# elun15/Graph-Convolutional-Network-for-Multi-Camera-Vehicle-Tracking

Measured on NVIDIA B200. Metric: mpn_inference_directed_edges_per_sec, higher is better.
Workload: dtype f32

## Files before the change

graph-convolutional-network-for-multi-camera-vehicle-tracking_b200/csrc/mpn_forward.cu:

```cuda
#include <mutex>
#include <new>
#include <stdlib.h>
#include <string.h>

#include "common.cuh"
#include "kernels.h"
#include "tcgen05.cuh"

namespace mpn {

enum {
  FC_ENC1_W = 0,
  FC_ENC1_C = 8,
  FC_ENC2_W = 12,
  FC_ENC2_C = 28,
  FC_EDGE_WE = 32,
  FC_BN3_S = 48,
  FC_BN3_T = 52,
  FC_NODE_WE = 64,
  FC_BN4_S = 192,
  FC_BN4_T = 224,
  FC_CLS_W = 256,
  FC_CLS_B = 264,
  FC_EDGE_WE0 = 272,
  FC_TOTAL = 288
};

constexpr int SUMS = MPN_SUMS_DOUBLES;
constexpr int SWEEP_THREADS = 256;
constexpr int SWEEP_BLOCKS_PER_SM = 4;
constexpr int SWEEP_GRID = kNumSMs * SWEEP_BLOCKS_PER_SM;
constexpr int SWEEP_RESIDENT_BLOCKS = 3;
constexpr int SWEEP_RESIDENT_GRID = kNumSMs * SWEEP_RESIDENT_BLOCKS;
constexpr float BN_EPS = 1e-5f;

struct EdgeConsts {
  float v[FC_TOTAL];
};

__device__ __forceinline__ void load_consts(EdgeConsts& sc, const float* __restrict__ consts) {
  for (int i = threadIdx.x; i < FC_TOTAL; i += blockDim.x) sc.v[i] = consts[i];
  __syncthreads();
}

constexpr int TASK_PART = 16;
__device__ __forceinline__ void warp_load_consts(EdgeConsts& sc, const float* __restrict__ consts_g, int lane) {
  __syncwarp();
  for (int i = lane; i < FC_TOTAL; i += 32) sc.v[i] = consts_g[i];
  __syncwarp();
}

__device__ __forceinline__ void enc_layer1(const EdgeConsts& sc, float2 ea, float (&a1)[4]) {
#pragma unroll
  for (int j = 0; j < 4; ++j)
    a1[j] = fmaxf(fmaf(sc.v[FC_ENC1_W + 2 * j], ea.x, fmaf(sc.v[FC_ENC1_W + 2 * j + 1], ea.y, sc.v[FC_ENC1_C + j])), 0.f);
}
__device__ __forceinline__ void enc_layer2_pre(const float* __restrict__ w2 , const float* __restrict__ c2,
                                               const float (&a1)[4], float (&u)[4]) {
#pragma unroll
  for (int j = 0; j < 4; ++j) {
// ... 494 lines not shown
    const float a_row = BATCHED ? 0.f : A[(size_t)tr.row * MPN_DH + lane];
    const float4 ps = (YSRC == 0) ? Ps[tr.row] : make_float4(0.f, 0.f, 0.f, 0.f);
    float s1[4] = {0.f, 0.f, 0.f, 0.f};
    float q[10] = {0.f, 0.f, 0.f, 0.f, 0.f, 0.f, 0.f, 0.f, 0.f, 0.f};
    for (int base = tr.beg; base < tr.end; base += 32 * U) {
      EdgeLoad<U> L;
      load_edges<U, YSRC == 0, YSRC == 0, YSRC == 1>(L, g, base, tr.end, lane, edge_attr, Pd, ybuf);
#pragma unroll
      for (int j = 0; j < U; ++j) {
        float ep[4];
        eprime_of<YSRC>(sc, ps, L.ea[j], L.pd[j], L.y[j], ep);
        if (!L.ok[j]) { ep[0] = ep[1] = ep[2] = ep[3] = 0.f; }
        int idx = 0;
#pragma unroll
        for (int a = 0; a < 4; ++a) {
          s1[a] += ep[a];
#pragma unroll
          for (int b = a; b < 4; ++b) { q[idx] = fmaf(ep[a], ep[b], q[idx]); ++idx; }
        }
      }
    }
#pragma unroll
    for (int a = 0; a < 4; ++a) s1[a] = warp_sum(s1[a]);
    if (lane == 0) s1_task[t] = make_float4(s1[0], s1[1], s1[2], s1[3]);
    if (!BATCHED) {
      const float nt = (float)(tr.end - tr.beg);
      const float4 wn = *reinterpret_cast<const float4*>(small + MPN_W_NODE_W + lane * 36 + 32);
      const float qd = fmaf(wn.x, s1[0], fmaf(wn.y, s1[1], fmaf(wn.z, s1[2], wn.w * s1[3])));
      m1 += (double)fmaf(nt, a_row, qd);
      m2 += (double)(a_row * fmaf(nt, a_row, 2.0f * qd));
    }
#pragma unroll
    for (int i = 0; i < 10; ++i) {
      const double v = warp_sum((double)q[i]);
      if (BATCHED) { if (lane == 0) partials[(size_t)t * TASK_PART + i] = v; }
      else if (lane == i) t2 += v;
    }
    tp.rotate(row_nn);
  }
  if (!BATCHED) {
    const int warp = threadIdx.x >> 5;
    red_m[warp][lane] = m1;
    red_m[warp][32 + lane] = m2;
    block_sum_lane_columns<10, SWEEP_THREADS>(t2, red, partials + (size_t)blockIdx.x * SUMS + 64);
    if (threadIdx.x < 64) {
      double sm = 0.0;
      for (int wv = 0; wv < SWEEP_THREADS / 32; ++wv) sm += red_m[wv][threadIdx.x];
      partials[(size_t)blockIdx.x * SUMS + threadIdx.x] = sm;
    }
    finalize_in_last_block(fin);
  }
}

template <bool MAXOP = false>
__device__ __forceinline__ float transpose_reduce32(float (&acc)[32], int lane) {
#pragma unroll
  for (int o = 16, n = 16; o > 0; o >>= 1, n >>= 1) {
    const bool upper = (lane & o) != 0;
#pragma unroll
    for (int i = 0; i < 16; ++i) {
      if (i < n) {
        const float send = upper ? acc[i] : acc[i + n];
        const float keep = upper ? acc[i + n] : acc[i];
        const float other = __shfl_xor_sync(0xffffffffu, send, o);
        acc[i] = MAXOP ? fmaxf(keep, other) : keep + other;
      }
    }
  }
  return acc[0];
}

typedef unsigned long long f32x2;
__device__ __forceinline__ f32x2 pack2(float lo, float hi) {
  f32x2 r;
  asm("mov.b64 %0, {%1, %2};" : "=l"(r) : "f"(lo), "f"(hi));
  return r;
}
__device__ __forceinline__ void unpack2(f32x2 v, float& lo, float& hi) { asm("mov.b64 {%0, %1}, %2;" : "=f"(lo), "=f"(hi) : "l"(v)); }
__device__ __forceinline__ f32x2 fma2(f32x2 a, f32x2 b, f32x2 c) {
  f32x2 d;
  asm("fma.rn.f32x2 %0, %1, %2, %3;" : "=l"(d) : "l"(a), "l"(b), "l"(c));
  return d;
}
__device__ __forceinline__ f32x2 add2(f32x2 a, f32x2 b) {
  f32x2 d;
  asm("add.rn.f32x2 %0, %1, %2;" : "=l"(d) : "l"(a), "l"(b));
  return d;
}
__device__ __forceinline__ f32x2 relu2(f32x2 v) {
  float lo, hi;
  unpack2(v, lo, hi);
  return pack2(fmaxf(lo, 0.f), fmaxf(hi, 0.f));
}

__global__ void __launch_bounds__(SWEEP_THREADS, 2) enc_moments1_packed_kernel(const float4* __restrict__ edge_attr2, long long n_pairs,
                                                                             const float2* __restrict__ edge_attr, long long E,
                                                                             const float* __restrict__ consts, const float* __restrict__ small,
                                                                             double* __restrict__ partials, const FinArgs fin) {
  pdl_wait();
  __shared__ EdgeConsts sc;
  __shared__ double red[(SWEEP_THREADS / 32) * 8];
  load_consts(sc, consts);
  f32x2 w1x[4], w1y[4], c1[4], w2[16], c2[4];
#pragma unroll
  for (int j = 0; j < 4; ++j) {
    w1x[j] = pack2(sc.v[FC_ENC1_W + 2 * j], sc.v[FC_ENC1_W + 2 * j]);
    w1y[j] = pack2(sc.v[FC_ENC1_W + 2 * j + 1], sc.v[FC_ENC1_W + 2 * j + 1]);
    c1[j] = pack2(sc.v[FC_ENC1_C + j], sc.v[FC_ENC1_C + j]);
    const float b = small[MPN_W_ENC2_B + j];
    c2[j] = pack2(b, b);
#pragma unroll
    for (int k = 0; k < 4; ++k) { const float w = small[MPN_W_ENC2_W + 4 * j + k]; w2[4 * j + k] = pack2(w, w); }
  }
// ... 126 lines not shown
      acc[p] = 0ull;
    }
    EdgeLoad<U> cur, nxt;
    load_edges<U, YSRC == 0, YSRC == 0, YSRC == 1>(cur, g, tr.beg, tr.end, lane, edge_attr, Pd, ybuf);
    for (int base = tr.beg; base < tr.end; base += 32 * U) {
      const int nbase = base + 32 * U;
      if (nbase < tr.end) load_edges<U, YSRC == 0, YSRC == 0, YSRC == 1>(nxt, g, nbase, tr.end, lane, edge_attr, Pd, ybuf);
      float ep[U][4];
      f32x2 ed[U][4];
#pragma unroll
      for (int j = 0; j < U; ++j) {
        eprime_of<YSRC>(sc, ps, cur.ea[j], cur.pd[j], cur.y[j], ep[j]);
#pragma unroll
        for (int k = 0; k < 4; ++k) ed[j][k] = pack2(ep[j][k], ep[j][k]);
      }
#pragma unroll
      for (int p = 0; p < 16; ++p) {
        ulonglong2 wa, wb;
        asm volatile("ld.shared.v2.b64 {%0, %1}, [%2];" : "=l"(wa.x), "=l"(wa.y) : "r"(w2_addr + p * 32));
        asm volatile("ld.shared.v2.b64 {%0, %1}, [%2];" : "=l"(wb.x), "=l"(wb.y) : "r"(w2_addr + p * 32 + 16));
#pragma unroll
        for (int j = 0; j < U; ++j) {
          f32x2 z = fma2(wa.x, ed[j][0], ap[p]);
          z = fma2(wa.y, ed[j][1], z);
          z = fma2(wb.x, ed[j][2], z);
          z = fma2(wb.y, ed[j][3], z);
          z = relu2(z);
          if (cur.ok[j]) {
            if (AGGMAX) {
              float zl, zh, al, ah;
              unpack2(z, zl, zh);
              unpack2(acc[p], al, ah);
              acc[p] = pack2(fmaxf(al, zl), fmaxf(ah, zh));
            } else {
              acc[p] = add2(acc[p], z);
            }
          }
        }
      }
#pragma unroll
      for (int j = 0; j < U; ++j)
        if (cur.ok[j]) classify_store<CLASSIFY>(sc, ep[j], cur.e[j], logits, pred, prob1);
#pragma unroll
      for (int j = 0; j < U; ++j) {
        cur.e[j] = nxt.e[j];
        cur.ok[j] = nxt.ok[j];
        if (YSRC == 0) { cur.ea[j] = nxt.ea[j]; cur.pd[j] = nxt.pd[j]; }
        else cur.y[j] = nxt.y[j];
      }
    }
    float accf[32];
#pragma unroll
    for (int p = 0; p < 16; ++p) unpack2(acc[p], accf[2 * p], accf[2 * p + 1]);
    const float total = transpose_reduce32<AGGMAX>(accf, lane);
    msg_task[(size_t)t * MPN_DH + lane] = total;
  }
}

constexpr int ATC_THREADS = 128;
constexpr int ATC_CTAS_PER_SM = 5;
constexpr int ATC_SEG = 128;
constexpr int ATC_BATCHES = 512;
constexpr int ATC_NB = 2;
constexpr int ATC_D = 4;
constexpr int ATC_RL = ATC_D + 1;
constexpr int ATC_SLOT_BYTES = 128 * 16;
__device__ __forceinline__ int tile_off(int row, int kcore) { return (row >> 3) * 64 + kcore * 32 + (row & 7) * 4; }
constexpr int ATC_GROUP_BYTES = 3 * 128;
constexpr int ATC_TILE_BYTES = 16 * ATC_GROUP_BYTES;
__device__ __forceinline__ void split_tf32(float v, float& hi, float& lo) {
  hi = __uint_as_float((__float_as_uint(v) + 0x1000u) & 0xffffe000u);
  lo = v - hi;
}
template <int BYTES>
__device__ __forceinline__ void cp_async(void* smem_dst, const void* gsrc) {
  asm volatile("cp.async.ca.shared.global [%0], [%1], %2;" ::"r"(smem_u32(smem_dst)), "l"(gsrc), "n"(BYTES) : "memory");
}
__device__ __forceinline__ void cp_async_commit() { asm volatile("cp.async.commit_group;" ::: "memory"); }
template <int N>
__device__ __forceinline__ void cp_async_wait() { asm volatile("cp.async.wait_group %0;" ::"n"(N) : "memory"); }
__device__ __forceinline__ uint32_t opaque_u32(uint32_t v) {
  asm volatile("" : "+r"(v));
  return v;
}
__device__ __forceinline__ void sts128(uint32_t addr, float a, float b, float c, float d) {
  asm volatile("st.shared.v4.f32 [%0], {%1, %2, %3, %4};" ::"r"(addr), "f"(a), "f"(b), "f"(c), "f"(d) : "memory");
}
__device__ __forceinline__ float4 lds128(uint32_t addr) {
  float4 v;
  asm volatile("ld.shared.v4.f32 {%0, %1, %2, %3}, [%4];" : "=f"(v.x), "=f"(v.y), "=f"(v.z), "=f"(v.w) : "r"(addr) : "memory");
  return v;
}

template <bool CLASSIFY, bool DECIDE, bool AGGMAX, int CTAS>
__global__ void __launch_bounds__(ATC_THREADS, CTAS) apply_tc_kernel(
    const mpn_graph g, const float4* __restrict__ ybuf, const float* __restrict__ A, const float* __restrict__ consts,
    float* __restrict__ msg_task, float2* __restrict__ logits, uint8_t* __restrict__ pred, float* __restrict__ prob1) {
  pdl_wait();
  __shared__ EdgeConsts sc;
  __shared__ __align__(128) float et[2 * ATC_NB][ATC_TILE_BYTES / 4];
  __shared__ __align__(128) float w1[32 * 8];
  __shared__ __align__(128) float w2[32 * 8];
  __shared__ __align__(16) float4 ring[ATC_RL][ATC_THREADS];
  __shared__ int s_row[ATC_SEG], s_beg[ATC_SEG], s_end[ATC_SEG];
  __shared__ int s_bstart[ATC_BATCHES], s_nbatch;
  __shared__ float red[2][ATC_THREADS / 32][32];
  __shared__ __align__(8) uint64_t bar;
  __shared__ uint32_t tmem_slot;
  load_consts(sc, consts);
  const int tid = threadIdx.x, lane = tid & 31, warp = tid >> 5;
  if (warp == 0) tmem_alloc(&tmem_slot, 32 * ATC_NB);
  if (tid == 0) {
    mbar_init(&bar, 1);
    asm volatile("fence.mbarrier_init.release.cluster;" ::: "memory");
  }
  if (tid < 32) {
    float wh[4], wl[4];
#pragma unroll
    for (int k = 0; k < 4; ++k) {
      split_tf32(sc.v[FC_NODE_WE + 4 * tid + k], wh[k], wl[k]);
      uint32_t lb;
      asm("cvt.rna.tf32.f32 %0, %1;" : "=r"(lb) : "f"(wl[k]));
      wl[k] = __uint_as_float(lb);
    }
    *reinterpret_cast<float4*>(&w1[tile_off(tid, 0)]) = make_float4(wh[0], wh[1], wh[2], wh[3]);
    *reinterpret_cast<float4*>(&w1[tile_off(tid, 1)]) = make_float4(wh[0], wh[1], wh[2], wh[3]);
    *reinterpret_cast<float4*>(&w2[tile_off(tid, 0)]) = make_float4(wl[0], wl[1], wl[2], wl[3]);
    *reinterpret_cast<float4*>(&w2[tile_off(tid, 1)]) = make_float4(0.f, 0.f, 0.f, 0.f);
  }
  tc_fence_before();
  __syncthreads();
  tc_fence_after();
  const uint32_t tmem = tmem_slot;
  constexpr uint32_t IDESC = make_idesc_tf32(128, 32);
  const uint64_t d_w1 = make_smem_desc_noswizzle(smem_u32(w1), 128, 256), d_w2 = make_smem_desc_noswizzle(smem_u32(w2), 128, 256);
  const uint64_t d_e1 = make_smem_desc_noswizzle(smem_u32(et[0]), 128, ATC_GROUP_BYTES);
  const uint64_t d_e2 = make_smem_desc_noswizzle(smem_u32(et[0]) + 128, 128, ATC_GROUP_BYTES);
  constexpr uint64_t BUF_STEP = ATC_TILE_BYTES >> 4;
  const uint32_t my_tmem = opaque_u32(tmem + ((uint32_t)(warp * 32) << 16));
  const uint32_t et_addr = opaque_u32(smem_u32(et[0]) + (uint32_t)((tid >> 3) * ATC_GROUP_BYTES + (tid & 7) * 16));
  const uint32_t ring_addr = opaque_u32(smem_u32(&ring[0][tid]));
  constexpr uint32_t TILE_BYTES = ATC_TILE_BYTES;
#pragma unroll
  for (int i = 0; i < 2 * ATC_NB; ++i)
    sts128(et_addr + (uint32_t)i * TILE_BYTES + 256, 1.f, 1.f, 0.f, 0.f);
  uint32_t phase = 0;
  const int n_tasks = *g.n_tasks;
  const int per = (n_tasks + (int)gridDim.x - 1) / (int)gridDim.x;
  const int t_first = blockIdx.x * per, t_last = min(n_tasks, t_first + per);
  const float bn_s = sc.v[FC_BN4_S + lane], bn_t = sc.v[FC_BN4_T + lane];
  const float s3[4] = {sc.v[FC_BN3_S], sc.v[FC_BN3_S + 1], sc.v[FC_BN3_S + 2], sc.v[FC_BN3_S + 3]};
  const float t3[4] = {sc.v[FC_BN3_T], sc.v[FC_BN3_T + 1], sc.v[FC_BN3_T + 2], sc.v[FC_BN3_T + 3]};
  int flushes = 0;

  const int seg_tasks = min(ATC_SEG, ATC_BATCHES / max(1, g.chunk / ATC_THREADS));
  for (int s0 = t_first; s0 < t_last; s0 += seg_tasks) {
    const int ns = min(seg_tasks, t_last - s0);
    __syncthreads();
    for (int i = tid; i < ns; i += ATC_THREADS) {
      const TaskRange tr = task_range(g, s0 + i);
      s_row[i] = tr.row; s_beg[i] = tr.beg; s_end[i] = tr.end;
    }
    __syncthreads();
    for (int i = tid; i < ns; i += ATC_THREADS) {
      int first = 0;
      for (int k = 0; k < i; ++k) first += (s_end[k] - s_beg[k] + ATC_THREADS - 1) / ATC_THREADS;
      const int nb_i = (s_end[i] - s_beg[i] + ATC_THREADS - 1) / ATC_THREADS;
      for (int k = 0; k < nb_i; ++k) s_bstart[first + k] = s_beg[i] + k * ATC_THREADS;
      if (i == ns - 1) s_nbatch = first + nb_i;
    }
    __syncthreads();
    const int n_batch = s_nbatch, seg_last = s_end[ns - 1] - 1;
    int st_j = 0, st_off = 0;
    auto issue_stream = [&]() {
      if (st_j < n_batch) {
        asm volatile("cp.async.ca.shared.global [%0], [%1], 16;" ::"r"(ring_addr + (uint32_t)st_off), "l"(ybuf + min(s_bstart[st_j] + tid, seg_last)) : "memory");
        ++st_j;
        st_off = (st_off == (ATC_RL - 1) * ATC_SLOT_BYTES) ? 0 : st_off + ATC_SLOT_BYTES;
      }
      cp_async_commit();
    };
#pragma unroll
    for (int j = 0; j < ATC_D; ++j) issue_stream();
    float acc[32];
#pragma unroll
    for (int c = 0; c < 32; ++c) acc[c] = 0.f;
    int pending = 0;
    int run_first = 0;
    int c_off = 0, buf = 0, issuer = 0;
    bool ok_prev[ATC_NB];
#pragma unroll
    for (int h = 0; h < ATC_NB; ++h) ok_prev[h] = false;
    float a_next = __ldg(A + (size_t)s_row[0] * MPN_DH + lane);
    auto drain = [&]() {
      mbar_wait(&bar, phase);
      phase ^= 1;
      tc_fence_after();
#pragma unroll
      for (int h = 0; h < ATC_NB; ++h) {
        if (h < pending) {
          float v[32];
          tmem_ld32(my_tmem + 32 * h, v);
          if (ok_prev[h]) {
#pragma unroll
            for (int c = 0; c < 32; ++c) acc[c] = AGGMAX ? fmaxf(acc[c], v[c]) : acc[c] + fabsf(v[c]);
          }
        }
      }
      tc_fence_before();
    };
    auto flush_to_red = [&]() {
      const float total = transpose_reduce32<AGGMAX>(acc, lane);
      red[flushes & 1][warp][lane] = total;
#pragma unroll
      for (int c = 0; c < 32; ++c) acc[c] = 0.f;
    };
    auto store_run = [&](int first, int last_t) {
      const float (*r)[32] = red[flushes & 1];
      msg_task[(size_t)(s0 + last_t) * MPN_DH + lane] = AGGMAX ? fmaxf(fmaxf(r[0][lane], r[1][lane]), fmaxf(r[2][lane], r[3][lane]))
                                                               : (r[0][lane] + r[1][lane]) + (r[2][lane] + r[3][lane]);
      for (int t = first; t < last_t; ++t) msg_task[(size_t)(s0 + t) * MPN_DH + lane] = 0.f;
    };
    for (int ti = 0; ti < ns; ++ti) {
      const int row = s_row[ti], t_beg = s_beg[ti], t_end = s_end[ti];
      const bool new_run = ti == 0 || row != s_row[ti - 1];
      const float a_cur = a_next;
      if (ti + 1 < ns) a_next = __ldg(A + (size_t)s_row[ti + 1] * MPN_DH + lane);
      for (int pos = t_beg; pos < t_end; pos += ATC_NB * ATC_THREADS) {
        const int nb = (pos + ATC_THREADS < t_end) ? ATC_NB : 1;
        bool ok[ATC_NB];
        float ep[ATC_NB][4];
#pragma unroll
        for (int h = 0; h < ATC_NB; ++h) {
          ok[h] = false;
          if (h < nb) {
            cp_async_wait<ATC_D - 1>();
            const float4 yv = lds128(ring_addr + (uint32_t)c_off);
            c_off = (c_off == (ATC_RL - 1) * ATC_SLOT_BYTES) ? 0 : c_off + ATC_SLOT_BYTES;
            issue_stream();
            const int e = pos + h * ATC_THREADS + tid;
            ok[h] = e < t_end;
            ep[h][0] = fmaxf(fmaf(s3[0], yv.x, t3[0]), 0.f);
            ep[h][1] = fmaxf(fmaf(s3[1], yv.y, t3[1]), 0.f);
            ep[h][2] = fmaxf(fmaf(s3[2], yv.z, t3[2]), 0.f);
            ep[h][3] = fmaxf(fmaf(s3[3], yv.w, t3[3]), 0.f);
            if (CLASSIFY && ok[h]) {
              float l0 = sc.v[FC_CLS_B + 0], l1 = sc.v[FC_CLS_B + 1];
#pragma unroll
              for (int k = 0; k < 4; ++k) {
                l0 = fmaf(sc.v[FC_CLS_W + k], ep[h][k], l0);
                l1 = fmaf(sc.v[FC_CLS_W + 4 + k], ep[h][k], l1);
              }
              logits[e] = make_float2(l0, l1);
              if (DECIDE) {
                pred[e] = (l1 > l0) ? 1 : 0;
                prob1[e] = softmax1(l0, l1);
              }
            }
            float eh[4], el[4];
#pragma unroll
            for (int k = 0; k < 4; ++k) split_tf32(ep[h][k], eh[k], el[k]);
            const uint32_t boff = (uint32_t)(buf * ATC_NB + h) * TILE_BYTES;
            sts128(et_addr + boff, el[0], el[1], el[2], el[3]);
            sts128(et_addr + boff + 128, eh[0], eh[1], eh[2], eh[3]);
          }
        }
        if (pending) drain();
#pragma unroll
        for (int h = 0; h < ATC_NB; ++h) ok_prev[h] = ok[h];
        const bool first_batch = pos == t_beg;
        const bool flushed = first_batch && new_run && ti > 0;
        if (first_batch && new_run) {
          if (ti > 0) flush_to_red();
          if (tid < 32) {
            float ah, al, al_hi, al_lo;
            split_tf32(fmaf(bn_s, a_cur, bn_t), ah, al);
            split_tf32(al, al_hi, al_lo);
            *reinterpret_cast<float4*>(&w2[tile_off(tid, 1)]) = make_float4(ah, al_hi, 0.f, 0.f);
          }
        }
        fence_proxy_async_smem();
        tc_fence_before();
        __syncthreads();
        if (tid == issuer) {
          tc_fence_after();
#pragma unroll
          for (int h = 0; h < ATC_NB; ++h) {
            if (h < nb) {
              umma_tf32(tmem + 32 * h, d_e1 + (uint64_t)(buf * ATC_NB + h) * BUF_STEP, d_w1, IDESC, 0);
              umma_tf32(tmem + 32 * h, d_e2 + (uint64_t)(buf * ATC_NB + h) * BUF_STEP, d_w2, IDESC, 1);
            }
          }
          umma_commit(&bar);
        }
        issuer = (issuer + 32) & (ATC_THREADS - 1);
        pending = nb;
        buf ^= 1;
        if (flushed) {
          if (warp == 0) store_run(run_first, ti - 1);
          ++flushes;
          run_first = ti;
        }
      }
    }
    if (pending) drain();
    flush_to_red();
    __syncthreads();
    if (warp == 0) store_run(run_first, ns - 1);
    ++flushes;
    cp_async_wait<0>();
  }
  tc_fence_before();
  __syncthreads();
  if (warp == 0) {
    tc_fence_after();
    tmem_dealloc(tmem, 32 * ATC_NB);
  }
}

template <int STAGE>
__global__ void __launch_bounds__(SWEEP_THREADS) enc_moments_task_kernel(const mpn_graph g, const float2* __restrict__ edge_attr,
                                                                         const float* __restrict__ consts, const float* __restrict__ small,
                                                                         double* __restrict__ task_part) {
  pdl_wait();
  __shared__ EdgeConsts scs[SWEEP_THREADS / 32];
  __shared__ float w2raw[20];
  if (threadIdx.x < 16) w2raw[threadIdx.x] = small[MPN_W_ENC2_W + threadIdx.x];
  else if (threadIdx.x < 20) w2raw[threadIdx.x] = small[MPN_W_ENC2_B + threadIdx.x - 16];
  __syncthreads();
  const int lane = threadIdx.x & 31;
  EdgeConsts& sc = scs[threadIdx.x >> 5];
  const int gwarp = (blockIdx.x * SWEEP_THREADS + threadIdx.x) >> 5;
  const int nwarps = (gridDim.x * SWEEP_THREADS) >> 5;
  const int n_tasks = *g.n_tasks;
  int cur_gid = -1;
  for (int t = gwarp; t < n_tasks; t += nwarps) {
    const TaskRange tr = task_range(g, t);
    if (STAGE == 1) {
      const int gid = g.node_gid[tr.row];
      if (gid != cur_gid) { warp_load_consts(sc, consts + (size_t)gid * FC_TOTAL, lane); cur_gid = gid; }
    }
    double acc[8] = {0, 0, 0, 0, 0, 0, 0, 0};
    for (int e = tr.beg + lane; e < tr.end; e += 32) {
      const float2 ea = ldg_stream2(edge_attr + e);
      if (STAGE == 0) {
        const double a = ea.x, b = ea.y;
        acc[0] += a; acc[1] += b; acc[2] += a * a; acc[3] += a * b; acc[4] += b * b;
      } else {
        float a1[4], u[4];
        enc_layer1(sc, ea, a1);
        enc_layer2_pre(w2raw, w2raw + 16, a1, u);
#pragma unroll
        for (int k = 0; k < 4; ++k) { const double d = u[k]; acc[k] += d; acc[4 + k] += d * d; }
      }
    }
#pragma unroll
    for (int k = 0; k < 8; ++k) {
      const double v = warp_sum(acc[k]);
      if (lane == 0) task_part[(size_t)t * TASK_PART + k] = v;
    }
  }
}

__global__ void __launch_bounds__(128) graph_finalize_kernel(int stage, const mpn_graph g, const double* __restrict__ task_part,
                                                             const float* __restrict__ A, const float4* __restrict__ s1_task,
                                                             const float* __restrict__ small, double* __restrict__ sums_all,
                                                             float* __restrict__ consts_all, int re_e) {
  pdl_wait();
  __shared__ double red[4][64];
// ... 688 lines not shown
    if (stage != MPN_STAGE_APPLY) {
      mpn::launch(graph_finalize_kernel, p->n_graphs, 128, 0, st, stage, g, tp, p->A, (const float4*)p->s1_task, p->w.small, p->sums, p->consts,
                                                         p->w.reattach_edges ? (stored ? 2 : 1) : 0);
      MPN_LAUNCH_OK();
    }
    return MPN_OK;
  }
  switch (stage) {
    case MPN_STAGE_ENC0:
      MPN_CUDA_OK(clear_moment_state(p, st));
      mpn::launch(enc_moments_kernel<0>, flat_grid, SWEEP_THREADS, 0, st, ea, g.n_edges, p->consts, p->w.small, p->partials, make_fin(p, stage, fused),
                  (const int*)nullptr);
      break;
    case MPN_STAGE_ENC1:
      if ((((uintptr_t)ea) & 15) == 0 && g.n_edges >= 2) {
        const long long n_pairs = g.n_edges >> 1;
        const int pgrid = (int)min((long long)kNumSMs * 2, (long long)div_up(n_pairs, SWEEP_THREADS));
        FinArgs pf;
        MPN_TRY(sweep_fin(p, stage, fused, pgrid, st, pf));
        mpn::launch(enc_moments1_packed_kernel, pgrid, SWEEP_THREADS, 0, st, (const float4*)ea, n_pairs, ea, g.n_edges, p->consts, p->w.small,
                    p->partials, pf);
      } else {
        mpn::launch(enc_moments_kernel<1>, flat_grid, SWEEP_THREADS, 0, st, ea, g.n_edges, p->consts, p->w.small, p->partials, make_fin(p, stage, fused),
                    (const int*)nullptr);
      }
      break;
    case MPN_STAGE_EDGE:
      if (step == 1) {
        if (stored) mpn::launch(edge_moments_kernel<0, true, false>, SWEEP_GRID, SWEEP_THREADS, 0, st, g, ea, Ps4, Pd4, yb, p->consts, p->partials, make_fin(p, stage, fused));
        else mpn::launch(edge_moments_kernel<0, false, false>, SWEEP_GRID, SWEEP_THREADS, 0, st, g, ea, Ps4, Pd4, nullptr, p->consts, p->partials, make_fin(p, stage, fused));
      } else {
        if (p->w.reattach_edges) mpn::launch(edge_moments_kernel<1, true, false, true>, SWEEP_GRID, SWEEP_THREADS, 0, st, g, ea, Ps4, Pd4, yb, p->consts, p->partials, make_fin(p, stage, fused));
        else mpn::launch(edge_moments_kernel<1, true, false>, SWEEP_GRID, SWEEP_THREADS, 0, st, g, ea, Ps4, Pd4, yb, p->consts, p->partials, make_fin(p, stage, fused));
      }
      break;
    case MPN_STAGE_NODE: {
      FinArgs nf;
      MPN_TRY(sweep_fin(p, stage, fused, stored ? SWEEP_RESIDENT_GRID : SWEEP_GRID, st, nf));
      if (stored) mpn::launch(node_moments_sweep_kernel<1, false>, SWEEP_RESIDENT_GRID, SWEEP_THREADS, 0, st, g, ea, Ps4, Pd4, yb, p->consts, (float4*)p->s1_task, p->partials, p->A, p->w.small, nf);
      else mpn::launch(node_moments_sweep_kernel<0, false>, SWEEP_GRID, SWEEP_THREADS, 0, st, g, ea, Ps4, Pd4, nullptr, p->consts, (float4*)p->s1_task, p->partials, p->A, p->w.small, nf);
      break;
    }
    case MPN_STAGE_APPLY: {
      const bool classify = logits_out != nullptr;
      float2* lg = (float2*)logits_out;
      if (p->L == 0) {
        MPN_REQUIRE(classify, "L == 0 needs a logits buffer");
        mpn::launch(classify_encoded_kernel, flat_grid, SWEEP_THREADS, 0, st, ea, g.n_edges, p->consts, lg, pred_out, prob1_out);
        break;
      }
      static int apply_tc = -1;
      if (apply_tc < 0) { const char* e = getenv("MPN_APPLY_TC"); apply_tc = e ? atoi(e) : 1; }
      p->msg_abs = 0;
      if (p->use_tc && apply_tc && stored && g.chunk >= ATC_THREADS && (!classify || (pred_out != nullptr) == (prob1_out != nullptr))) {
        const bool agg_max = p->w.node_agg == MPN_AGG_MAX;
        p->msg_abs = agg_max ? 0 : 1;
#define MPN_ATC3(CL, DE, MX, NC) mpn::launch(apply_tc_kernel<CL, DE, MX, NC>, kNumSMs * NC, ATC_THREADS, 0, st, g, yb, p->A, p->consts, p->msg_task, lg, pred_out, prob1_out)
#define MPN_ATC2(CL, DE, MX) MPN_ATC3(CL, DE, MX, ATC_CTAS_PER_SM)
#define MPN_ATC(CL, DE) do { if (agg_max) MPN_ATC2(CL, DE, true); else MPN_ATC2(CL, DE, false); } while (0)
        if (!classify) MPN_ATC(false, false);
        else if (pred_out && prob1_out) MPN_ATC(true, true);
        else MPN_ATC(true, false);
#undef MPN_ATC
#undef MPN_ATC2
#undef MPN_ATC3
        break;
      }
#define MPN_APPLY2(YS, CL, MX) mpn::launch(apply_kernel<YS, CL, false, MX>, SWEEP_GRID, SWEEP_THREADS, 0, st, g, ea, Ps4, Pd4, yb, p->A, p->consts, p->msg_task, lg, pred_out, prob1_out)
#define MPN_APPLY(YS, CL) do { if (p->w.node_agg == MPN_AGG_MAX) MPN_APPLY2(YS, CL, true); else MPN_APPLY2(YS, CL, false); } while (0)
      if (stored) { if (classify) MPN_APPLY(1, true); else MPN_APPLY(1, false); }
      else        { if (classify) MPN_APPLY(0, true); else MPN_APPLY(0, false); }
#undef MPN_APPLY
#undef MPN_APPLY2
      break;
    }
    default:
      MPN_REQUIRE(false, "unknown stage %d", stage);
  }
  MPN_LAUNCH_OK();
  return MPN_OK;
}

int mpn_plan_finalize(mpn_fwd_plan* p, int32_t step, int32_t stage, void* stream) {
  MPN_REQUIRE(p, "finalize: NULL plan");
  (void)step;
  if (p->n_graphs > 1) return MPN_OK;
  mpn::launch(finalize_kernel, 1, FIN_THREADS, 0, (cudaStream_t)stream, make_fin(p, stage, false), 0, 1);
  MPN_LAUNCH_OK();
  return MPN_OK;
}

int mpn_plan_reduce(mpn_fwd_plan* p, int32_t stage, int with_consts, void* stream) {
  MPN_REQUIRE(p, "reduce: NULL plan");
  if (p->n_graphs > 1) return MPN_OK;
  mpn::launch(finalize_kernel, 1, FIN_THREADS, 0, (cudaStream_t)stream, make_fin(p, stage, false), 1, with_consts);
  MPN_LAUNCH_OK();
  return MPN_OK;
}

int mpn_plan_node_finalize(mpn_fwd_plan* p, int32_t step, void* stream) {
  MPN_REQUIRE(p, "node_finalize: NULL plan");
  (void)step;
  mpn::launch(node_finalize_kernel<false>, min(kNumSMs * 8, div_up((long long)p->g.n_nodes * 32, 256)), 256, 0, (cudaStream_t)stream, p->g, p->msg_task, p->h_full, PeerArgs(), abs_fix(p));
  MPN_LAUNCH_OK();
  return MPN_OK;
}

struct SideStream {
  cudaStream_t stream;
  cudaEvent_t fork, join;
};
static SideStream* side_stream() {
  static SideStream table[64];
  static int state[64];
  static std::mutex init_lock;
  int dev = 0;
  if (cudaGetDevice(&dev) != cudaSuccess || dev < 0 || dev >= 64) return nullptr;
  std::lock_guard<std::mutex> hold(init_lock);
// ... 364 lines not shown
```

Measured before the change: 21.45 billion.

## Replace tcgen05/TMEM apply kernel with per-warp mma.sync TF32 kernel

Replaces the block-level tcgen05 UMMA apply kernel, which staged edges through cp.async rings, TMEM accumulators, mbarriers and block-wide syncs, with a warp-independent kernel. Each warp handles one task at a time using mma.sync m16n8k8 TF32, with the split hi/lo operands staged through a small per-warp smem slab. Reduction is done in registers with a smaller transpose reduce. This removes block synchronisation and TMEM round trips. In exchange it gives up the larger UMMA tiles and adds more per-warp shuffles and shared-memory traffic. The launch condition is also relaxed, and the DECIDE path is now chosen when either pred or prob1 is provided.

Result: slower. 21.24 billion (median of 6 runs) (-1.0%).

```diff
diff --git a/graph-convolutional-network-for-multi-camera-vehicle-tracking_b200/csrc/mpn_forward.cu b/graph-convolutional-network-for-multi-camera-vehicle-tracking_b200/csrc/mpn_forward.cu
--- a/graph-convolutional-network-for-multi-camera-vehicle-tracking_b200/csrc/mpn_forward.cu
+++ b/graph-convolutional-network-for-multi-camera-vehicle-tracking_b200/csrc/mpn_forward.cu
@@ -5,7 +5,6 @@
 
 #include "common.cuh"
 #include "kernels.h"
-#include "tcgen05.cuh"
 
 namespace mpn {
 
@@ -606,13 +605,13 @@
   }
 }
 
-template <bool MAXOP = false>
-__device__ __forceinline__ float transpose_reduce32(float (&acc)[32], int lane) {
-#pragma unroll
-  for (int o = 16, n = 16; o > 0; o >>= 1, n >>= 1) {
+template <int N, bool MAXOP = false>
+__device__ __forceinline__ float transpose_reduce(float (&acc)[N], int lane) {
+#pragma unroll
+  for (int o = 16, n = N / 2; n > 0; o >>= 1, n >>= 1) {
     const bool upper = (lane & o) != 0;
 #pragma unroll
-    for (int i = 0; i < 16; ++i) {
+    for (int i = 0; i < N / 2; ++i) {
       if (i < n) {
         const float send = upper ? acc[i] : acc[i + n];
         const float keep = upper ? acc[i + n] : acc[i];
@@ -845,269 +844,148 @@
     float accf[32];
 #pragma unroll
     for (int p = 0; p < 16; ++p) unpack2(acc[p], accf[2 * p], accf[2 * p + 1]);
-    const float total = transpose_reduce32<AGGMAX>(accf, lane);
+    const float total = transpose_reduce<32, AGGMAX>(accf, lane);
     msg_task[(size_t)t * MPN_DH + lane] = total;
   }
 }
 
-constexpr int ATC_THREADS = 128;
-constexpr int ATC_CTAS_PER_SM = 5;
-constexpr int ATC_SEG = 128;
-constexpr int ATC_BATCHES = 512;
-constexpr int ATC_NB = 2;
-constexpr int ATC_D = 4;
-constexpr int ATC_RL = ATC_D + 1;
-constexpr int ATC_SLOT_BYTES = 128 * 16;
-__device__ __forceinline__ int tile_off(int row, int kcore) { return (row >> 3) * 64 + kcore * 32 + (row & 7) * 4; }
-constexpr int ATC_GROUP_BYTES = 3 * 128;
-constexpr int ATC_TILE_BYTES = 16 * ATC_GROUP_BYTES;
 __device__ __forceinline__ void split_tf32(float v, float& hi, float& lo) {
   hi = __uint_as_float((__float_as_uint(v) + 0x1000u) & 0xffffe000u);
   lo = v - hi;
 }
-template <int BYTES>
-__device__ __forceinline__ void cp_async(void* smem_dst, const void* gsrc) {
-  asm volatile("cp.async.ca.shared.global [%0], [%1], %2;" ::"r"(smem_u32(smem_dst)), "l"(gsrc), "n"(BYTES) : "memory");
-}
-__device__ __forceinline__ void cp_async_commit() { asm volatile("cp.async.commit_group;" ::: "memory"); }
-template <int N>
-__device__ __forceinline__ void cp_async_wait() { asm volatile("cp.async.wait_group %0;" ::"n"(N) : "memory"); }
-__device__ __forceinline__ uint32_t opaque_u32(uint32_t v) {
-  asm volatile("" : "+r"(v));
-  return v;
-}
-__device__ __forceinline__ void sts128(uint32_t addr, float a, float b, float c, float d) {
-  asm volatile("st.shared.v4.f32 [%0], {%1, %2, %3, %4};" ::"r"(addr), "f"(a), "f"(b), "f"(c), "f"(d) : "memory");
-}
-__device__ __forceinline__ float4 lds128(uint32_t addr) {
-  float4 v;
-  asm volatile("ld.shared.v4.f32 {%0, %1, %2, %3}, [%4];" : "=f"(v.x), "=f"(v.y), "=f"(v.z), "=f"(v.w) : "r"(addr) : "memory");
-  return v;
-}
-
-template <bool CLASSIFY, bool DECIDE, bool AGGMAX, int CTAS>
-__global__ void __launch_bounds__(ATC_THREADS, CTAS) apply_tc_kernel(
+__device__ __forceinline__ void mma_tf32(float (&d)[4], const uint32_t (&a)[4], uint32_t b0, uint32_t b1) {
+  asm("mma.sync.aligned.m16n8k8.row.col.f32.tf32.tf32.f32 {%0, %1, %2, %3}, {%4, %5, %6, %7}, {%8, %9}, {%0, %1, %2, %3};"
+      : "+f"(d[0]), "+f"(d[1]), "+f"(d[2]), "+f"(d[3])
+      : "r"(a[0]), "r"(a[1]), "r"(a[2]), "r"(a[3]), "r"(b0), "r"(b1));
+}
+
+#ifndef AMMA_L2PF
+#define AMMA_L2PF 0
+#endif
+constexpr int AMMA_U = 2;
+constexpr int AMMA_ROW = 12;
+
+template <bool CLASSIFY, bool DECIDE, bool AGGMAX>
+__global__ void __launch_bounds__(SWEEP_THREADS, SWEEP_RESIDENT_BLOCKS) apply_mma_kernel(
     const mpn_graph g, const float4* __restrict__ ybuf, const float* __restrict__ A, const float* __restrict__ consts,
     float* __restrict__ msg_task, float2* __restrict__ logits, uint8_t* __restrict__ pred, float* __restrict__ prob1) {
   pdl_wait();
-  __shared__ EdgeConsts sc;
-  __shared__ __align__(128) float et[2 * ATC_NB][ATC_TILE_BYTES / 4];
-  __shared__ __align__(128) float w1[32 * 8];
-  __shared__ __align__(128) float w2[32 * 8];
-  __shared__ __align__(16) float4 ring[ATC_RL][ATC_THREADS];
-  __shared__ int s_row[ATC_SEG], s_beg[ATC_SEG], s_end[ATC_SEG];
-  __shared__ int s_bstart[ATC_BATCHES], s_nbatch;
-  __shared__ float red[2][ATC_THREADS / 32][32];
-  __shared__ __align__(8) uint64_t bar;
-  __shared__ uint32_t tmem_slot;
+  constexpr int U = AMMA_U;
+  __shared__ __align__(16) EdgeConsts sc;
+  __shared__ __align__(16) float slab_all[SWEEP_THREADS / 32][32 * U * AMMA_ROW];
   load_consts(sc, consts);
-  const int tid = threadIdx.x, lane = tid & 31, warp = tid >> 5;
-  if (warp == 0) tmem_alloc(&tmem_slot, 32 * ATC_NB);
-  if (tid == 0) {
-    mbar_init(&bar, 1);
-    asm volatile("fence.mbarrier_init.release.cluster;" ::: "memory");
-  }
-  if (tid < 32) {
-    float wh[4], wl[4];
-#pragma unroll
-    for (int k = 0; k < 4; ++k) {
-      split_tf32(sc.v[FC_NODE_WE + 4 * tid + k], wh[k], wl[k]);
-      uint32_t lb;
-      asm("cvt.rna.tf32.f32 %0, %1;" : "=r"(lb) : "f"(wl[k]));
-      wl[k] = __uint_as_float(lb);
-    }
-    *reinterpret_cast<float4*>(&w1[tile_off(tid, 0)]) = make_float4(wh[0], wh[1], wh[2], wh[3]);
-    *reinterpret_cast<float4*>(&w1[tile_off(tid, 1)]) = make_float4(wh[0], wh[1], wh[2], wh[3]);
-    *reinterpret_cast<float4*>(&w2[tile_off(tid, 0)]) = make_float4(wl[0], wl[1], wl[2], wl[3]);
-    *reinterpret_cast<float4*>(&w2[tile_off(tid, 1)]) = make_float4(0.f, 0.f, 0.f, 0.f);
-  }
-  tc_fence_before();
-  __syncthreads();
-  tc_fence_after();
-  const uint32_t tmem = tmem_slot;
-  constexpr uint32_t IDESC = make_idesc_tf32(128, 32);
-  const uint64_t d_w1 = make_smem_desc_noswizzle(smem_u32(w1), 128, 256), d_w2 = make_smem_desc_noswizzle(smem_u32(w2), 128, 256);
-  const uint64_t d_e1 = make_smem_desc_noswizzle(smem_u32(et[0]), 128, ATC_GROUP_BYTES);
-  const uint64_t d_e2 = make_smem_desc_noswizzle(smem_u32(et[0]) + 128, 128, ATC_GROUP_BYTES);
-  constexpr uint64_t BUF_STEP = ATC_TILE_BYTES >> 4;
-  const uint32_t my_tmem = opaque_u32(tmem + ((uint32_t)(warp * 32) << 16));
-  const uint32_t et_addr = opaque_u32(smem_u32(et[0]) + (uint32_t)((tid >> 3) * ATC_GROUP_BYTES + (tid & 7) * 16));
-  const uint32_t ring_addr = opaque_u32(smem_u32(&ring[0][tid]));
-  constexpr uint32_t TILE_BYTES = ATC_TILE_BYTES;
-#pragma unroll
-  for (int i = 0; i < 2 * ATC_NB; ++i)
-    sts128(et_addr + (uint32_t)i * TILE_BYTES + 256, 1.f, 1.f, 0.f, 0.f);
-  uint32_t phase = 0;
+  const int lane = threadIdx.x & 31;
+  const int gq = lane >> 2, tq = lane & 3;
+  float* slab = slab_all[threadIdx.x >> 5];
+  uint32_t bh[4], bl[4];
+#pragma unroll
+  for (int j = 0; j < 4; ++j) {
+    float wh, wl;
+    split_tf32(sc.v[FC_NODE_WE + 4 * (8 * j + gq) + tq], wh, wl);
+    asm("cvt.rna.tf32.f32 %0, %1;" : "=r"(bl[j]) : "f"(wl));
+    bh[j] = __float_as_uint(wh);
+  }
+  const float one = tq < 2 ? 1.f : 0.f;
+  const uint32_t st_addr = (uint32_t)__cvta_generic_to_shared(slab + lane * AMMA_ROW);
+  const uint32_t ld_addr = (uint32_t)__cvta_generic_to_shared(slab + gq * AMMA_ROW + tq);
+
+  const int gwarp = (blockIdx.x * SWEEP_THREADS + threadIdx.x) >> 5;
+  const int nwarps = (gridDim.x * SWEEP_THREADS) >> 5;
   const int n_tasks = *g.n_tasks;
-  const int per = (n_tasks + (int)gridDim.x - 1) / (int)gridDim.x;
-  const int t_first = blockIdx.x * per, t_last = min(n_tasks, t_first + per);
-  const float bn_s = sc.v[FC_BN4_S + lane], bn_t = sc.v[FC_BN4_T + lane];
-  const float s3[4] = {sc.v[FC_BN3_S], sc.v[FC_BN3_S + 1], sc.v[FC_BN3_S + 2], sc.v[FC_BN3_S + 3]};
-  const float t3[4] = {sc.v[FC_BN3_T], sc.v[FC_BN3_T + 1], sc.v[FC_BN3_T + 2], sc.v[FC_BN3_T + 3]};
-  int flushes = 0;
-
-  const int seg_tasks = min(ATC_SEG, ATC_BATCHES / max(1, g.chunk / ATC_THREADS));
-  for (int s0 = t_first; s0 < t_last; s0 += seg_tasks) {
-    const int ns = min(seg_tasks, t_last - s0);
-    __syncthreads();
-    for (int i = tid; i < ns; i += ATC_THREADS) {
-      const TaskRange tr = task_range(g, s0 + i);
-      s_row[i] = tr.row; s_beg[i] = tr.beg; s_end[i] = tr.end;
-    }
-    __syncthreads();
-    for (int i = tid; i < ns; i += ATC_THREADS) {
-      int first = 0;
-      for (int k = 0; k < i; ++k) first += (s_end[k] - s_beg[k] + ATC_THREADS - 1) / ATC_THREADS;
-      const int nb_i = (s_end[i] - s_beg[i] + ATC_THREADS - 1) / ATC_THREADS;
-      for (int k = 0; k < nb_i; ++k) s_bstart[first + k] = s_beg[i] + k * ATC_THREADS;
-      if (i == ns - 1) s_nbatch = first + nb_i;
-    }
-    __syncthreads();
-    const int n_batch = s_nbatch, seg_last = s_end[ns - 1] - 1;
-    int st_j = 0, st_off = 0;
-    auto issue_stream = [&]() {
-      if (st_j < n_batch) {
-        asm volatile("cp.async.ca.shared.global [%0], [%1], 16;" ::"r"(ring_addr + (uint32_t)st_off), "l"(ybuf + min(s_bstart[st_j] + tid, seg_last)) : "memory");
-        ++st_j;
-        st_off = (st_off == (ATC_RL - 1) * ATC_SLOT_BYTES) ? 0 : st_off + ATC_SLOT_BYTES;
-      }
-      cp_async_commit();
-    };
-#pragma unroll
-    for (int j = 0; j < ATC_D; ++j) issue_stream();
-    float acc[32];
-#pragma unroll
-    for (int c = 0; c < 32; ++c) acc[c] = 0.f;
-    int pending = 0;
-    int run_first = 0;
-    int c_off = 0, buf = 0, issuer = 0;
-    bool ok_prev[ATC_NB];
-#pragma unroll
-    for (int h = 0; h < ATC_NB; ++h) ok_prev[h] = false;
-    float a_next = __ldg(A + (size_t)s_row[0] * MPN_DH + lane);
-    auto drain = [&]() {
-      mbar_wait(&bar, phase);
-      phase ^= 1;
-      tc_fence_after();
-#pragma unroll
-      for (int h = 0; h < ATC_NB; ++h) {
-        if (h < pending) {
-          float v[32];
-          tmem_ld32(my_tmem + 32 * h, v);
-          if (ok_prev[h]) {
-#pragma unroll
-            for (int c = 0; c < 32; ++c) acc[c] = AGGMAX ? fmaxf(acc[c], v[c]) : acc[c] + fabsf(v[c]);
+  const int t_last = gwarp + max(n_tasks - 1 - gwarp, 0) / nwarps * nwarps;
+  if (!task_in(t_last, n_tasks)) return;
+  TaskPrefetch tp;
+  tp.start(g, t_last, -nwarps, n_tasks);
+  float4 ynx[U];
+#pragma unroll
+  for (int j = 0; j < U; ++j) ynx[j] = ybuf[min(tp.cur.beg + 32 * j + lane, tp.cur.end - 1)];
+  float a_next = A[(size_t)tp.cur.row * MPN_DH + lane];
+  for (int t = t_last; task_in(t, n_tasks); t -= nwarps) {
+    const int row_nn = tp.issue(g, t, -nwarps, n_tasks);
+    const TaskRange tr = tp.cur;
+    const bool has_next = task_in(t - nwarps, n_tasks);
+    float ah, al, al_hi, al_lo;
+    split_tf32(fmaf(sc.v[FC_BN4_S + lane], a_next, sc.v[FC_BN4_T + lane]), ah, al);
+    split_tf32(al, al_hi, al_lo);
+    if (has_next) a_next = A[(size_t)tp.nxt.row * MPN_DH + lane];
+    uint32_t ba[4];
+#pragma unroll
+    for (int j = 0; j < 4; ++j) {
+      const float xh = __shfl_sync(0xffffffffu, ah, 8 * j + gq), xl = __shfl_sync(0xffffffffu, al_hi, 8 * j + gq);
+      ba[j] = __float_as_uint(tq == 0 ? xh : (tq == 1 ? xl : 0.f));
+    }
+    float acc[8] = {0.f, 0.f, 0.f, 0.f, 0.f, 0.f, 0.f, 0.f};
+    for (int base = tr.beg; base < tr.end; base += 32 * U) {
+      const bool more = base + 32 * U < tr.end;
+      const int nbase = more ? base + 32 * U : tp.nxt.beg, nend = more ? tr.end : tp.nxt.end;
+#if AMMA_L2PF
+      {
+        int pb = nbase + 32 * U, pe = nend;
+        bool pv = more || has_next;
+        if (more && pb >= pe) { pb = tp.nxt.beg; pe = tp.nxt.end; pv = has_next; }
+        if (pv && pb < pe) {
+#pragma unroll
+          for (int j = 0; j < U; ++j) asm volatile("prefetch.global.L2 [%0];" ::"l"(ybuf + min(pb + 32 * j + lane, pe - 1)));
+        }
+      }
+#endif
+      __syncwarp();
+#pragma unroll
+      for (int j = 0; j < U; ++j) {
+        const float4 yv = ynx[j];
+        if (more || has_next) ynx[j] = ybuf[min(nbase + 32 * j + lane, nend - 1)];
+        const int e = base + 32 * j + lane;
+        const bool ok = e < tr.end;
+        const float4 s3 = *reinterpret_cast<const float4*>(&sc.v[FC_BN3_S]), t3 = *reinterpret_cast<const float4*>(&sc.v[FC_BN3_T]);
+        float ep[4];
+        ep[0] = fmaxf(fmaf(s3.x, yv.x, t3.x), 0.f);
+        ep[1] = fmaxf(fmaf(s3.y, yv.y, t3.y), 0.f);
+        ep[2] = fmaxf(fmaf(s3.z, yv.z, t3.z), 0.f);
+        ep[3] = fmaxf(fmaf(s3.w, yv.w, t3.w), 0.f);
+        if (ok) classify_store<CLASSIFY>(sc, ep, e, logits, DECIDE ? pred : nullptr, DECIDE ? prob1 : nullptr);
+        float eh[4], el[4];
+#pragma unroll
+        for (int k = 0; k < 4; ++k) {
+          split_tf32(ok ? ep[k] : 0.f, eh[k], el[k]);
+        }
+        const uint32_t a = st_addr + j * 32 * AMMA_ROW * 4;
+        asm volatile("st.shared.v4.f32 [%0], {%1, %2, %3, %4};" ::"r"(a), "f"(el[0]), "f"(el[1]), "f"(el[2]), "f"(el[3]) : "memory");
+        asm volatile("st.shared.v4.f32 [%0], {%1, %2, %3, %4};" ::"r"(a + 16), "f"(eh[0]), "f"(eh[1]), "f"(eh[2]), "f"(eh[3]) : "memory");
+      }
+      __syncwarp();
+      const int n_ok = tr.end - base;
+#pragma unroll
+      for (int m = 0; m < 2 * U; ++m) {
+        if (16 * m < n_ok) {
+          const uint32_t a = ld_addr + m * 16 * AMMA_ROW * 4;
+          uint32_t e1[4], e2[4];
+          asm volatile("ld.shared.b32 %0, [%1];" : "=r"(e1[0]) : "r"(a) : "memory");
+          asm volatile("ld.shared.b32 %0, [%1];" : "=r"(e1[1]) : "r"(a + 8 * AMMA_ROW * 4) : "memory");
+          asm volatile("ld.shared.b32 %0, [%1];" : "=r"(e1[2]) : "r"(a + 16) : "memory");
+          asm volatile("ld.shared.b32 %0, [%1];" : "=r"(e1[3]) : "r"(a + 8 * AMMA_ROW * 4 + 16) : "memory");
+          e2[0] = e1[2];
+          e2[1] = e1[3];
+          e2[2] = __float_as_uint(16 * m + gq < n_ok ? one : 0.f);
+          e2[3] = __float_as_uint(16 * m + gq + 8 < n_ok ? one : 0.f);
+#pragma unroll
+          for (int j = 0; j < 4; ++j) {
+            float z[4] = {0.f, 0.f, 0.f, 0.f};
+            mma_tf32(z, e1, bh[j], bh[j]);
+            mma_tf32(z, e2, bl[j], ba[j]);
+            if (AGGMAX) {
+              acc[2 * j] = fmaxf(acc[2 * j], fmaxf(z[0], z[2]));
+              acc[2 * j + 1] = fmaxf(acc[2 * j + 1], fmaxf(z[1], z[3]));
+            } else {
+              acc[2 * j] = acc[2 * j] + fabsf(z[0]) + fabsf(z[2]);
+              acc[2 * j + 1] = acc[2 * j + 1] + fabsf(z[1]) + fabsf(z[3]);
+            }
           }
         }
       }
-      tc_fence_before();
-    };
-    auto flush_to_red = [&]() {
-      const float total = transpose_reduce32<AGGMAX>(acc, lane);
-      red[flushes & 1][warp][lane] = total;
-#pragma unroll
-      for (int c = 0; c < 32; ++c) acc[c] = 0.f;
-    };
-    auto store_run = [&](int first, int last_t) {
-      const float (*r)[32] = red[flushes & 1];
-      msg_task[(size_t)(s0 + last_t) * MPN_DH + lane] = AGGMAX ? fmaxf(fmaxf(r[0][lane], r[1][lane]), fmaxf(r[2][lane], r[3][lane]))
-                                                               : (r[0][lane] + r[1][lane]) + (r[2][lane] + r[3][lane]);
-      for (int t = first; t < last_t; ++t) msg_task[(size_t)(s0 + t) * MPN_DH + lane] = 0.f;
-    };
-    for (int ti = 0; ti < ns; ++ti) {
-      const int row = s_row[ti], t_beg = s_beg[ti], t_end = s_end[ti];
-      const bool new_run = ti == 0 || row != s_row[ti - 1];
-      const float a_cur = a_next;
-      if (ti + 1 < ns) a_next = __ldg(A + (size_t)s_row[ti + 1] * MPN_DH + lane);
-      for (int pos = t_beg; pos < t_end; pos += ATC_NB * ATC_THREADS) {
-        const int nb = (pos + ATC_THREADS < t_end) ? ATC_NB : 1;
-        bool ok[ATC_NB];
-        float ep[ATC_NB][4];
-#pragma unroll
-        for (int h = 0; h < ATC_NB; ++h) {
-          ok[h] = false;
-          if (h < nb) {
-            cp_async_wait<ATC_D - 1>();
-            const float4 yv = lds128(ring_addr + (uint32_t)c_off);
-            c_off = (c_off == (ATC_RL - 1) * ATC_SLOT_BYTES) ? 0 : c_off + ATC_SLOT_BYTES;
-            issue_stream();
-            const int e = pos + h * ATC_THREADS + tid;
-            ok[h] = e < t_end;
-            ep[h][0] = fmaxf(fmaf(s3[0], yv.x, t3[0]), 0.f);
-            ep[h][1] = fmaxf(fmaf(s3[1], yv.y, t3[1]), 0.f);
-            ep[h][2] = fmaxf(fmaf(s3[2], yv.z, t3[2]), 0.f);
-            ep[h][3] = fmaxf(fmaf(s3[3], yv.w, t3[3]), 0.f);
-            if (CLASSIFY && ok[h]) {
-              float l0 = sc.v[FC_CLS_B + 0], l1 = sc.v[FC_CLS_B + 1];
-#pragma unroll
-              for (int k = 0; k < 4; ++k) {
-                l0 = fmaf(sc.v[FC_CLS_W + k], ep[h][k], l0);
-                l1 = fmaf(sc.v[FC_CLS_W + 4 + k], ep[h][k], l1);
-              }
-              logits[e] = make_float2(l0, l1);
-              if (DECIDE) {
-                pred[e] = (l1 > l0) ? 1 : 0;
-                prob1[e] = softmax1(l0, l1);
-              }
-            }
-            float eh[4], el[4];
-#pragma unroll
-            for (int k = 0; k < 4; ++k) split_tf32(ep[h][k], eh[k], el[k]);
-            const uint32_t boff = (uint32_t)(buf * ATC_NB + h) * TILE_BYTES;
-            sts128(et_addr + boff, el[0], el[1], el[2], el[3]);
-            sts128(et_addr + boff + 128, eh[0], eh[1], eh[2], eh[3]);
-          }
-        }
-        if (pending) drain();
-#pragma unroll
-        for (int h = 0; h < ATC_NB; ++h) ok_prev[h] = ok[h];
-        const bool first_batch = pos == t_beg;
-        const bool flushed = first_batch && new_run && ti > 0;
-        if (first_batch && new_run) {
-          if (ti > 0) flush_to_red();
-          if (tid < 32) {
-            float ah, al, al_hi, al_lo;
-            split_tf32(fmaf(bn_s, a_cur, bn_t), ah, al);
-            split_tf32(al, al_hi, al_lo);
-            *reinterpret_cast<float4*>(&w2[tile_off(tid, 1)]) = make_float4(ah, al_hi, 0.f, 0.f);
-          }
-        }
-        fence_proxy_async_smem();
-        tc_fence_before();
-        __syncthreads();
-        if (tid == issuer) {
-          tc_fence_after();
-#pragma unroll
-          for (int h = 0; h < ATC_NB; ++h) {
-            if (h < nb) {
-              umma_tf32(tmem + 32 * h, d_e1 + (uint64_t)(buf * ATC_NB + h) * BUF_STEP, d_w1, IDESC, 0);
-              umma_tf32(tmem + 32 * h, d_e2 + (uint64_t)(buf * ATC_NB + h) * BUF_STEP, d_w2, IDESC, 1);
-            }
-          }
-          umma_commit(&bar);
-        }
-        issuer = (issuer + 32) & (ATC_THREADS - 1);
-        pending = nb;
-        buf ^= 1;
-        if (flushed) {
-          if (warp == 0) store_run(run_first, ti - 1);
-          ++flushes;
-          run_first = ti;
-        }
-      }
-    }
-    if (pending) drain();
-    flush_to_red();
-    __syncthreads();
-    if (warp == 0) store_run(run_first, ns - 1);
-    ++flushes;
-    cp_async_wait<0>();
-  }
-  tc_fence_before();
-  __syncthreads();
-  if (warp == 0) {
-    tc_fence_after();
-    tmem_dealloc(tmem, 32 * ATC_NB);
+    }
+    const float total = transpose_reduce<8, AGGMAX>(acc, lane);
+    msg_task[(size_t)t * MPN_DH + 8 * (gq >> 1) + 2 * tq + (gq & 1)] = total;
+    tp.rotate(row_nn);
   }
 }
 
@@ -1902,18 +1780,16 @@
       static int apply_tc = -1;
       if (apply_tc < 0) { const char* e = getenv("MPN_APPLY_TC"); apply_tc = e ? atoi(e) : 1; }
       p->msg_abs = 0;
-      if (p->use_tc && apply_tc && stored && g.chunk >= ATC_THREADS && (!classify || (pred_out != nullptr) == (prob1_out != nullptr))) {
+      if (p->use_tc && apply_tc && stored && g.chunk >= 128) {
         const bool agg_max = p->w.node_agg == MPN_AGG_MAX;
         p->msg_abs = agg_max ? 0 : 1;
-#define MPN_ATC3(CL, DE, MX, NC) mpn::launch(apply_tc_kernel<CL, DE, MX, NC>, kNumSMs * NC, ATC_THREADS, 0, st, g, yb, p->A, p->consts, p->msg_task, lg, pred_out, prob1_out)
-#define MPN_ATC2(CL, DE, MX) MPN_ATC3(CL, DE, MX, ATC_CTAS_PER_SM)
-#define MPN_ATC(CL, DE) do { if (agg_max) MPN_ATC2(CL, DE, true); else MPN_ATC2(CL, DE, false); } while (0)
-        if (!classify) MPN_ATC(false, false);
-        else if (pred_out && prob1_out) MPN_ATC(true, true);
-        else MPN_ATC(true, false);
-#undef MPN_ATC
-#undef MPN_ATC2
-#undef MPN_ATC3
+#define MPN_AMMA2(CL, DE, MX) mpn::launch(apply_mma_kernel<CL, DE, MX>, SWEEP_RESIDENT_GRID, SWEEP_THREADS, 0, st, g, yb, p->A, p->consts, p->msg_task, lg, pred_out, prob1_out)
+#define MPN_AMMA(CL, DE) do { if (agg_max) MPN_AMMA2(CL, DE, true); else MPN_AMMA2(CL, DE, false); } while (0)
+        if (!classify) MPN_AMMA(false, false);
+        else if (pred_out || prob1_out) MPN_AMMA(true, true);
+        else MPN_AMMA(true, false);
+#undef MPN_AMMA
+#undef MPN_AMMA2
         break;
       }
 #define MPN_APPLY2(YS, CL, MX) mpn::launch(apply_kernel<YS, CL, false, MX>, SWEEP_GRID, SWEEP_THREADS, 0, st, g, ea, Ps4, Pd4, yb, p->A, p->consts, p->msg_task, lg, pred_out, prob1_out)
```
